# rapidsai/cugraph

Measured on NVIDIA B200. Metric: MTEPS (million traversed edges/sec) PageRank RMAT-24 ef-16, 100 iterations, higher is better.
Workload: dtype f32

## Files before the change

### cugraph_b200/csrc/pagerank.cu

```cuda
#include "sweep.cuh"

#include <algorithm>
#include <cmath>
#include <cstring>

namespace b200 {
namespace {

constexpr int kBlock = 256;
inline int grid_for(int64_t n) { return (int)std::min<int64_t>(std::max<int64_t>((n + kBlock - 1) / kBlock, 1), 1 << 22); }

template <typename T>
__global__ void k_fill(T* a, int32_t n, T v)
{
  int i = blockIdx.x * blockDim.x + threadIdx.x;
  if (i < n) a[i] = v;
}

__global__ void k_out_degree(int32_t const* __restrict__ indices, long long nnz, int32_t* __restrict__ deg)
{
  for (long long i = blockIdx.x * (long long)blockDim.x + threadIdx.x; i < nnz; i += (long long)gridDim.x * blockDim.x)
    atomicAdd(deg + indices[i], 1);
}

template <typename T>
__global__ void k_out_weight(int32_t const* __restrict__ indices, T const* __restrict__ w, long long nnz, double* __restrict__ sums)
{
  for (long long i = blockIdx.x * (long long)blockDim.x + threadIdx.x; i < nnz; i += (long long)gridDim.x * blockDim.x)
    atomicAdd(sums + indices[i], (double)w[i]);
}

template <typename S, typename T>
__global__ void k_cast(S const* in, int32_t n, T* out)
{
  int i = blockIdx.x * blockDim.x + threadIdx.x;
  if (i < n) out[i] = (T)in[i];
}

__device__ __forceinline__ double block_sum(double v, double* smem)
{
  v = warp_sum(v);
  if ((threadIdx.x & 31) == 0) smem[threadIdx.x >> 5] = v;
  __syncthreads();
  double t = 0.0;
  if (threadIdx.x < 32) {
    t = (threadIdx.x < (blockDim.x >> 5)) ? smem[threadIdx.x] : 0.0;
    t = warp_sum(t);
  }
  __syncthreads();
  return t;
}

template <typename T>
__global__ void __launch_bounds__(kBlock)
k_vertex_pass(T const* __restrict__ pr_new, T const* __restrict__ pr_old, T const* __restrict__ out_w,
              T* __restrict__ x, int32_t n, pr_state_t* __restrict__ st)
{
  if (st->done) return;
  __shared__ double smem[8];
  double diff = 0.0, dang = 0.0;
  for (int i = blockIdx.x * blockDim.x + threadIdx.x; i < n; i += gridDim.x * blockDim.x) {
    T nv = pr_new[i];
    T ow = out_w[i];
    if (pr_old) diff += fabs((double)nv - (double)pr_old[i]);
    if (ow == (T)0) dang += (double)nv;
    x[i] = (ow == (T)0) ? nv : nv / ow;
  }
  diff = block_sum(diff, smem);
  dang = block_sum(dang, smem);
  if (threadIdx.x == 0) {
    if (pr_old) atomicAdd(&st->diff, diff);
    atomicAdd(&st->dangling, dang);
  }
}

__global__ void k_finalize(pr_state_t* st, double alpha, double epsilon, int n_vertices, int personalized,
                           int count_iteration, int max_iterations)
{
  if (st->done) return;
  double base    = st->dangling * alpha + (1.0 - alpha);
  st->init       = personalized ? 0.0 : base / (double)n_vertices;
  st->pers_scale = base;
  if (count_iteration) {
    st->iter += 1;
    st->last_diff = st->diff;
    if (st->diff < epsilon || st->iter >= max_iterations) st->done = 1;
  }
  st->diff     = 0.0;
  st->dangling = 0.0;
}

template <typename T>
__global__ void k_personalize(int32_t const* __restrict__ pv, T const* __restrict__ pvals, int32_t n, double pers_sum,
                              T* __restrict__ y, pr_state_t const* __restrict__ st)
{
  if (st->done) return;
  int i = blockIdx.x * blockDim.x + threadIdx.x;
  if (i < n) y[pv[i]] = (T)((double)y[pv[i]] + st->pers_scale * ((double)pvals[i] / pers_sum));
}

template <typename T>
__global__ void k_sum(T const* a, int32_t n, double* out)
{
  __shared__ double smem[8];
  double s = 0.0;
  for (int i = blockIdx.x * blockDim.x + threadIdx.x; i < n; i += gridDim.x * blockDim.x) s += (double)a[i];
  s = block_sum(s, smem);
  if (threadIdx.x == 0) atomicAdd(out, s);
}

template <typename T>
__global__ void k_count_negative(T const* a, int64_t n, int* out)
{
  for (int64_t i = blockIdx.x * (int64_t)blockDim.x + threadIdx.x; i < n; i += (int64_t)gridDim.x * blockDim.x)
    if (a[i] < (T)0) atomicAdd(out, 1);
}

template <typename T>
__global__ void k_fill_pattern(T* x, int32_t n)
{
  int i = blockIdx.x * blockDim.x + threadIdx.x;
  if (i < n) x[i] = (T)(0.5 + (double)((unsigned)(i * 2654435761u) >> 16) / 65536.0);
}

template <typename O, typename T>
__global__ void k_compare_rows(O const* __restrict__ off, int32_t const* __restrict__ row_vertex, T const* __restrict__ a,
                               T const* __restrict__ b, int32_t n_rows, int32_t n_hi, double tol,
                               unsigned long long* __restrict__ worst , unsigned long long* __restrict__ n_bad )
{
  int r = blockIdx.x * blockDim.x + threadIdx.x;
  if (r >= n_rows) return;
  const int v        = row_vertex ? row_vertex[r] : r;
  const double va = (double)a[v], vb = (double)b[v];
  const double den   = fmax(fabs(va), 1e-300);
  const float rel    = (float)fmin(fabs(va - vb) / den, 1e30);
  const int cls      = r < n_hi ? 0 : 1;
  atomicMax(worst + cls, ((unsigned long long)__float_as_uint(rel) << 32) | (unsigned)r);
  if (rel > tol) atomicAdd(n_bad + cls, 1ull);
  (void)off;
}

struct pr_args {
  device_array_view_impl const* pre_v{nullptr};
  device_array_view_impl const* pre_w{nullptr};
  device_array_view_impl const* init_v{nullptr};
  device_array_view_impl const* init_val{nullptr};
  device_array_view_impl const* pers_v{nullptr};
  device_array_view_impl const* pers_val{nullptr};
  double alpha{0.85};
  double epsilon{1e-5};
  size_t max_iterations{100};
  bool expensive{false};
};

template <typename T>
void pagerank_typed(handle_impl const& h, graph_impl& g, pr_args const& a, centrality_result_impl& res)
{
  phase_trace tr(h);
  const int32_t nv = g.n_vertices;
  B200_EXPECTS(a.alpha >= 0.0 && a.alpha <= 1.0, CUGRAPH_UNKNOWN_ERROR, "Invalid input argument: alpha should be in [0.0, 1.0].");
  B200_EXPECTS(a.epsilon >= 0.0, CUGRAPH_UNKNOWN_ERROR, "Invalid input argument: epsilon should be non-negative.");
  if (nv == 0) {
    res.vertices   = new device_array_impl{dbuf(0, h.stream), 0, g.vertex_type};
    res.values     = new device_array_impl{dbuf(0, h.stream), 0, g.weight_type};
    res.iterations = 0;
    res.converged  = true;
    return;
  }
  csx_t const& c = pull_view(h, g);
  B200_EXPECTS(c.degree_sorted, CUGRAPH_UNKNOWN_ERROR, "internal: pull view is not binned");
  const bool weighted = g.weighted;

  dbuf out_w_user;
  T const* out_w = nullptr;
  if (a.pre_w) {
    out_w_user = collect_vertex_values<T>(h, g, a.pre_v, a.pre_w, (T)0);
    out_w      = out_w_user.as<T>();
  } else {
    if (c.out_w.data() == nullptr) {
      dbuf ow = make_dbuf<T>(nv, h.stream);
      if (weighted) {
        dbuf sums = make_dbuf<double>(nv, h.stream);
        CUDA_TRY(cudaMemsetAsync(sums.data(), 0, sizeof(double) * nv, h.stream));
        if (c.nnz > 0)
          B200_LAUNCH(h, (k_out_weight<T>), std::min(grid_for(c.nnz), 148 * 16), kBlock, 0, c.indices.as<int32_t>(),
                      c.weights.as<T>(), (long long)c.nnz, sums.as<double>());
        B200_LAUNCH(h, (k_cast<double, T>), grid_for(nv), kBlock, 0, sums.as<double>(), nv, ow.as<T>());
      } else {
        dbuf deg = make_dbuf<int32_t>(nv, h.stream);
        CUDA_TRY(cudaMemsetAsync(deg.data(), 0, sizeof(int32_t) * nv, h.stream));
        if (c.nnz > 0)
          B200_LAUNCH(h, k_out_degree, std::min(grid_for(c.nnz), 148 * 16), kBlock, 0, c.indices.as<int32_t>(),
                      (long long)c.nnz, deg.as<int32_t>());
        B200_LAUNCH(h, (k_cast<int32_t, T>), grid_for(nv), kBlock, 0, deg.as<int32_t>(), nv, ow.as<T>());
      }
      sync(h);
      c.out_w = std::move(ow);
    }
    out_w = c.out_w.as<T>();
  }
  tr.mark("pagerank: pull view + out-weights");
  if (a.expensive && weighted && c.nnz > 0) {
    dbuf neg = make_dbuf<int>(1, h.stream);
    CUDA_TRY(cudaMemsetAsync(neg.data(), 0, sizeof(int), h.stream));
    B200_LAUNCH(h, (k_count_negative<T>), std::min(grid_for(c.nnz), 148 * 16), kBlock, 0, c.weights.as<T>(), c.nnz, neg.as<int>());
    int hneg = 0;
    CUDA_TRY(cudaMemcpyAsync(&hneg, neg.data(), sizeof(int), cudaMemcpyDeviceToHost, h.stream));
    sync(h);
    B200_EXPECTS(hneg == 0, CUGRAPH_UNKNOWN_ERROR, "Invalid input argument: input edge weights should have non-negative values.");
  }

  dbuf pers_idx, pers_vals;
  int32_t n_pers  = 0;
  double pers_sum = 0.0;
  if (a.pers_v) {
    B200_EXPECTS(a.pers_val && a.pers_v->size == a.pers_val->size, CUGRAPH_UNKNOWN_ERROR,
                 "Invalid input argument: if personalization.has_value() is true, the size of vertices and values should match");
    B200_EXPECTS(a.pers_v->size > 0, CUGRAPH_UNKNOWN_ERROR,
                 "Invalid input argument: if personalizations.has_value() is true, the input personalization vector size should not be 0.");
    n_pers   = (int32_t)a.pers_v->size;
    pers_idx = make_dbuf<int32_t>(n_pers, h.stream);
    ext_to_int(h, g, a.pers_v->data, n_pers, pers_idx.as<int32_t>());
    dbuf bad = make_dbuf<int>(1, h.stream);
    CUDA_TRY(cudaMemsetAsync(bad.data(), 0, sizeof(int), h.stream));
    B200_LAUNCH(h, (k_count_negative<int32_t>), grid_for(n_pers), kBlock, 0, pers_idx.as<int32_t>(), (int64_t)n_pers, bad.as<int>());
    dbuf dsum = make_dbuf<double>(1, h.stream);
    CUDA_TRY(cudaMemsetAsync(dsum.data(), 0, sizeof(double), h.stream));
    B200_LAUNCH(h, (k_sum<T>), std::min(grid_for(n_pers), 1024), kBlock, 0, (T const*)a.pers_val->data, n_pers, dsum.as<double>());
    int hbad = 0;
    CUDA_TRY(cudaMemcpyAsync(&hbad, bad.data(), sizeof(int), cudaMemcpyDeviceToHost, h.stream));
    CUDA_TRY(cudaMemcpyAsync(&pers_sum, dsum.data(), sizeof(double), cudaMemcpyDeviceToHost, h.stream));
    sync(h);
    B200_EXPECTS(hbad == 0, CUGRAPH_INVALID_INPUT, "Invalid input argument: peresonalization vertices have invalid vertex IDs.");
    B200_EXPECTS(pers_sum > 0.0, CUGRAPH_UNKNOWN_ERROR, "Invalid input argument: sum of personalization valuese should be positive.");
  }

  dbuf pr_a = make_dbuf<T>(nv, h.stream), pr_b = make_dbuf<T>(nv, h.stream);
  dbuf x    = make_dbuf<T>(padded_x_elems(nv, sizeof(T)), h.stream);
  CUDA_TRY(cudaMemsetAsync(x.data(), 0, padded_x_elems(nv, sizeof(T)) * sizeof(T), h.stream));
  dbuf acc_hi = make_dbuf<double>(acc_rows(c), h.stream);
  CUDA_TRY(cudaMemsetAsync(acc_hi.data(), 0, sizeof(double) * acc_rows(c), h.stream));
  dbuf state = make_dbuf<pr_state_t>(1, h.stream);
  CUDA_TRY(cudaMemsetAsync(state.data(), 0, sizeof(pr_state_t), h.stream));
  pr_state_t* st = state.as<pr_state_t>();

  if (a.init_val) {
    dbuf guess = collect_vertex_values<T>(h, g, a.init_v, a.init_val, (T)0);
    CUDA_TRY(cudaMemcpyAsync(pr_a.data(), guess.data(), sizeof(T) * nv, cudaMemcpyDeviceToDevice, h.stream));
    sync(h);
  } else {
    B200_LAUNCH(h, (k_fill<T>), grid_for(nv), kBlock, 0, pr_a.as<T>(), nv, (T)((T)1 / (T)nv));
  }

  tr.mark("pagerank: state setup");
  const int vgrid = std::min(grid_for(nv), h.sm_count * 8);
  const int max_it = (int)std::min<size_t>(a.max_iterations, 0x7fffffff);
  B200_LAUNCH(h, (k_vertex_pass<T>), vgrid, kBlock, 0, pr_a.as<T>(), (T const*)nullptr, out_w, x.as<T>(), nv, st);
  B200_LAUNCH(h, k_finalize, 1, 1, 0, st, a.alpha, a.epsilon, nv, n_pers > 0 ? 1 : 0, 0, max_it);

  T* cur = pr_a.as<T>();
  T* nxt = pr_b.as<T>();
  pr_state_t* hst = reinterpret_cast<pr_state_t*>(h.pinned);
  int enqueued    = 0;
  int iters       = 0;
  const int batch = (a.epsilon > 0.0) ? 8 : 64;
  if (max_it == 0) {
  }
  while (true) {
    int todo = std::min(batch, std::max(max_it, 1) - enqueued);
    for (int k = 0; k < todo; ++k) {
      if (c.offs64) launch_pull_sweep<int64_t, T>(h, c, x.as<T>(), nxt, acc_hi.as<double>(), a.alpha, st);
      else launch_pull_sweep_auto<int32_t, T>(h, c, nv, x.as<T>(), nxt, acc_hi.as<double>(), a.alpha, st);
      if (n_pers > 0)
        B200_LAUNCH(h, (k_personalize<T>), grid_for(n_pers), kBlock, 0, pers_idx.as<int32_t>(), (T const*)a.pers_val->data,
                    n_pers, pers_sum, nxt, st);
      B200_LAUNCH(h, (k_vertex_pass<T>), vgrid, kBlock, 0, nxt, cur, out_w, x.as<T>(), nv, st);
      B200_LAUNCH(h, k_finalize, 1, 1, 0, st, a.alpha, a.epsilon, nv, n_pers > 0 ? 1 : 0, 1, max_it);
      std::swap(cur, nxt);
      ++enqueued;
    }
    check_last("pagerank iteration");
    CUDA_TRY(cudaMemcpyAsync(hst, st, sizeof(pr_state_t), cudaMemcpyDeviceToHost, h.stream));
    sync(h);
    iters = hst->iter;
    if (hst->done || enqueued >= std::max(max_it, 1)) break;
  }
  tr.mark("pagerank: iterations (+ layout staging on the first call)");
  T* final_pr = (iters % 2 == 0) ? pr_a.as<T>() : pr_b.as<T>();

  res.vertices   = new device_array_impl{reported_vertices(h, g), (size_t)nv, g.vertex_type};
  res.values     = new device_array_impl{to_reported_order(h, g, final_pr, sizeof(T)), (size_t)nv, g.weight_type};
  res.iterations = (size_t)iters;
  res.converged  = (size_t)iters < a.max_iterations;
  sync(h);
  tr.mark("pagerank: result gather");
}

cugraph_error_code_t pagerank_entry(const cugraph_resource_handle_t* handle, cugraph_graph_t* graph, pr_args a,
                                    bool require_convergence, cugraph_centrality_result_t** result,
                                    cugraph_error_t** error)
{
  return guarded(error, [&] {
    auto const& h = H(handle);
    auto* g       = G(graph);
    B200_EXPECTS(result != nullptr, CUGRAPH_INVALID_INPUT, "result out-pointer is NULL");
    *result = nullptr;
    if (a.pre_v) {
      B200_EXPECTS(a.pre_v->type == g->vertex_type, CUGRAPH_INVALID_INPUT,
                   "vertex type of graph and precomputed_vertex_out_weight_vertices must match");
      B200_EXPECTS(a.pre_w && a.pre_w->type == g->weight_type, CUGRAPH_INVALID_INPUT,
                   "vertex type of graph and precomputed_vertex_out_weight_sums must match");
    }
    if (a.init_v) {
      B200_EXPECTS(a.init_v->type == g->vertex_type, CUGRAPH_INVALID_INPUT,
                   "vertex type of graph and initial_guess_vertices must match");
      B200_EXPECTS(a.init_val && a.init_val->type == g->weight_type, CUGRAPH_INVALID_INPUT,
                   "vertex type of graph and initial_guess_values must match");
    }
    if (a.pers_v) {
      B200_EXPECTS(a.pers_v->type == g->vertex_type, CUGRAPH_INVALID_INPUT,
                   "vertex type of graph and personalization_vector must match");
      B200_EXPECTS(a.pers_val && a.pers_val->type == g->weight_type, CUGRAPH_INVALID_INPUT,
                   "vertex type of graph and personalization_vector must match");
    }
    if (!a.pre_w) a.pre_v = nullptr;
    if (!a.init_val) a.init_v = nullptr;
    auto res = std::make_unique<centrality_result_impl>();
    if (g->mg) {
      mg_pagerank(h, *g, mg_pr_args{a.alpha, a.epsilon, a.max_iterations}, *res);
    } else if (g->weight_type == FLOAT32) {
      pagerank_typed<float>(h, *g, a, *res);
    } else {
      pagerank_typed<double>(h, *g, a, *res);
    }
    bool converged = res->converged;
    *result        = reinterpret_cast<cugraph_centrality_result_t*>(res.release());
    B200_EXPECTS(!require_convergence || converged, CUGRAPH_UNKNOWN_ERROR, "PageRank failed to converge.");
  });
}

}

}

using namespace b200;

extern "C" {

cugraph_type_erased_device_array_view_t* cugraph_centrality_result_get_vertices(cugraph_centrality_result_t* result)
{
  auto* r = reinterpret_cast<centrality_result_impl*>(result);
  return reinterpret_cast<cugraph_type_erased_device_array_view_t*>(r->vertices->new_view());
}

cugraph_type_erased_device_array_view_t* cugraph_centrality_result_get_values(cugraph_centrality_result_t* result)
{
  auto* r = reinterpret_cast<centrality_result_impl*>(result);
  return reinterpret_cast<cugraph_type_erased_device_array_view_t*>(r->values->new_view());
}

size_t cugraph_centrality_result_get_num_iterations(cugraph_centrality_result_t* result)
{
  return reinterpret_cast<centrality_result_impl*>(result)->iterations;
}

bool_t cugraph_centrality_result_converged(cugraph_centrality_result_t* result)
{
  return reinterpret_cast<centrality_result_impl*>(result)->converged ? TRUE : FALSE;
}

void cugraph_centrality_result_free(cugraph_centrality_result_t* result)
{
  if (!result) return;
  auto* r = reinterpret_cast<centrality_result_impl*>(result);
  delete r->vertices;
  delete r->values;
  delete r;
}

#define PR_ARGS_COMMON                                                                          \
  pr_args a;                                                                                    \
  a.pre_v          = V(precomputed_vertex_out_weight_vertices);                                 \
  a.pre_w          = V(precomputed_vertex_out_weight_sums);                                     \
  a.init_v         = V(initial_guess_vertices);                                                 \
  a.init_val       = V(initial_guess_values);                                                   \
  a.alpha          = alpha;                                                                     \
  a.epsilon        = epsilon;                                                                   \
  a.max_iterations = max_iterations;                                                            \
  a.expensive      = do_expensive_check == TRUE;

cugraph_error_code_t cugraph_pagerank(const cugraph_resource_handle_t* handle, cugraph_graph_t* graph,
                                      const cugraph_type_erased_device_array_view_t* precomputed_vertex_out_weight_vertices,
                                      const cugraph_type_erased_device_array_view_t* precomputed_vertex_out_weight_sums,
                                      const cugraph_type_erased_device_array_view_t* initial_guess_vertices,
                                      const cugraph_type_erased_device_array_view_t* initial_guess_values, double alpha,
                                      double epsilon, size_t max_iterations, bool_t do_expensive_check,
                                      cugraph_centrality_result_t** result, cugraph_error_t** error)
{
  PR_ARGS_COMMON
  return pagerank_entry(handle, graph, a, true, result, error);
}

cugraph_error_code_t cugraph_pagerank_allow_nonconvergence(
  const cugraph_resource_handle_t* handle, cugraph_graph_t* graph,
  const cugraph_type_erased_device_array_view_t* precomputed_vertex_out_weight_vertices,
  const cugraph_type_erased_device_array_view_t* precomputed_vertex_out_weight_sums,
  const cugraph_type_erased_device_array_view_t* initial_guess_vertices,
  const cugraph_type_erased_device_array_view_t* initial_guess_values, double alpha, double epsilon,
  size_t max_iterations, bool_t do_expensive_check, cugraph_centrality_result_t** result, cugraph_error_t** error)
{
  PR_ARGS_COMMON
  return pagerank_entry(handle, graph, a, false, result, error);
}

cugraph_error_code_t cugraph_personalized_pagerank(
  const cugraph_resource_handle_t* handle, cugraph_graph_t* graph,
  const cugraph_type_erased_device_array_view_t* precomputed_vertex_out_weight_vertices,
  const cugraph_type_erased_device_array_view_t* precomputed_vertex_out_weight_sums,
  const cugraph_type_erased_device_array_view_t* initial_guess_vertices,
  const cugraph_type_erased_device_array_view_t* initial_guess_values,
  const cugraph_type_erased_device_array_view_t* personalization_vertices,
  const cugraph_type_erased_device_array_view_t* personalization_values, double alpha, double epsilon,
  size_t max_iterations, bool_t do_expensive_check, cugraph_centrality_result_t** result, cugraph_error_t** error)
{
  PR_ARGS_COMMON
  a.pers_v   = V(personalization_vertices);
  a.pers_val = V(personalization_values);
  return pagerank_entry(handle, graph, a, true, result, error);
}

// ... 106 lines not shown
```

### cugraph_b200/csrc/spmv.cuh

```cuda
#pragma once
#include "graph.cuh"

#include <cstdlib>

namespace b200 {

struct pr_state_t {
  double diff;
  double dangling;
  double init;
  double pers_scale;
  double last_diff;
  int iter;
  int done;
};

#ifndef B200_HOST_EMU
__device__ __forceinline__ int ld_stream(const int* p)
{
  int v;
  asm volatile("ld.global.nc.L1::no_allocate.s32 %0, [%1];" : "=r"(v) : "l"(p));
  return v;
}
__device__ __forceinline__ float ld_stream(const float* p)
{
  float v;
  asm volatile("ld.global.nc.L1::no_allocate.f32 %0, [%1];" : "=f"(v) : "l"(p));
  return v;
}
__device__ __forceinline__ double ld_stream(const double* p)
{
  double v;
  asm volatile("ld.global.nc.L1::no_allocate.f64 %0, [%1];" : "=d"(v) : "l"(p));
  return v;
}
#else
inline int ld_stream(const int* p) { return *p; }
inline float ld_stream(const float* p) { return *p; }
inline double ld_stream(const double* p) { return *p; }
#endif

__device__ __forceinline__ double warp_sum(double v)
{
#pragma unroll
  for (int o = 16; o > 0; o >>= 1) v += __shfl_xor_sync(0xffffffffu, v, o);
  return v;
}

template <typename O, typename T, bool WEIGHTED>
__global__ void __launch_bounds__(256)
k_spmv_hi(O const* __restrict__ offsets, int32_t const* __restrict__ indices, T const* __restrict__ weights,
          T const* __restrict__ x, T* __restrict__ y, int32_t const* __restrict__ row_vertex,
          int32_t const* __restrict__ chunk_first_row, int32_t n_chunks, long long nnz_hi,
          double* __restrict__ acc_hi, double alpha, pr_state_t const* __restrict__ st)
{
  if (st->done) return;
  const int lane = threadIdx.x & 31;
  const int c    = (int)((blockIdx.x * (long long)blockDim.x + threadIdx.x) >> 5);
  if (c >= n_chunks) return;
  const double init  = st->init;
  const long long e0 = (long long)c * kWarpChunk;
  const long long e1 = (e0 + kWarpChunk < nnz_hi) ? e0 + kWarpChunk : nnz_hi;
  int r              = chunk_first_row[c];
  long long row_beg  = (long long)offsets[r];
  long long row_end  = (long long)offsets[r + 1];
  long long e        = e0;
  while (e < e1) {
    const long long seg_end = row_end < e1 ? row_end : e1;
    double acc              = 0.0;
    long long i             = e + lane;
    for (; i + 96 < seg_end; i += 128) {
      int s0 = ld_stream(indices + i), s1 = ld_stream(indices + i + 32);
      int s2 = ld_stream(indices + i + 64), s3 = ld_stream(indices + i + 96);
      T x0 = x[s0], x1 = x[s1], x2 = x[s2], x3 = x[s3];
      if (WEIGHTED) {
        x0 *= ld_stream(weights + i);
        x1 *= ld_stream(weights + i + 32);
        x2 *= ld_stream(weights + i + 64);
        x3 *= ld_stream(weights + i + 96);
      }
      acc += ((double)x0 + (double)x1) + ((double)x2 + (double)x3);
    }
    for (; i < seg_end; i += 32) {
      T xv = x[ld_stream(indices + i)];
      if (WEIGHTED) xv *= ld_stream(weights + i);
      acc += (double)xv;
    }
    acc = warp_sum(acc);
    if (lane == 0) {
      const bool whole = (row_beg >= e0) && (row_end <= e1);
      if (whole) {
        const int v = row_vertex ? row_vertex[r] : r;
        y[v]        = (T)(acc * alpha + init);
      } else {
        atomicAdd(acc_hi + r, acc);
      }
    }
    e = seg_end;
    if (e == row_end && e < e1) {
      ++r;
      row_beg = row_end;
      row_end = (long long)offsets[r + 1];
    }
  }
}

template <typename T>
__global__ void k_spmv_hi_finish(int32_t const* __restrict__ split_rows, int32_t n_split, double* __restrict__ acc_hi,
                                 T* __restrict__ y, int32_t const* __restrict__ row_vertex, double alpha,
                                 pr_state_t const* __restrict__ st)
{
  if (st->done) return;
  int k = blockIdx.x * blockDim.x + threadIdx.x;
  if (k >= n_split) return;
  int r     = split_rows[k];
  int v     = row_vertex ? row_vertex[r] : r;
  y[v]      = (T)(acc_hi[r] * alpha + st->init);
  acc_hi[r] = 0.0;
}

struct low_bins_t {
  int32_t row_begin[kNumSeg];
  int32_t block_begin[kNumSeg];
};

__host__ __device__ __forceinline__ int low_bin_lanes(int b) { return b == 0 ? 4 : (b == 1 ? 2 : 1); }

template <typename O, typename T, bool WEIGHTED>
__global__ void __launch_bounds__(256)
k_spmv_low(O const* __restrict__ offsets, int32_t const* __restrict__ indices, T const* __restrict__ weights,
           T const* __restrict__ x, T* __restrict__ y, int32_t const* __restrict__ row_vertex, low_bins_t bins,
           double alpha, pr_state_t const* __restrict__ st)
{
  if (st->done) return;
  int b = 0;
#pragma unroll
  for (int k = 1; k < kNumSeg - 1; ++k)
    if ((int)blockIdx.x >= bins.block_begin[k]) b = k;
  const double init = st->init;
  const int blk     = blockIdx.x - bins.block_begin[b];
  if (b == kNumSeg - 2) {
    int r = bins.row_begin[b] + blk * 256 + threadIdx.x;
    if (r < bins.row_begin[b + 1]) y[row_vertex ? row_vertex[r] : r] = (T)init;
    return;
  }
  const int g   = low_bin_lanes(b);
  const int sub = threadIdx.x & (g - 1);
  const int r   = bins.row_begin[b] + blk * (256 / g) + (threadIdx.x / g);
  double acc    = 0.0;
  const bool in = r < bins.row_begin[b + 1];
  if (in) {
    const long long lo = (long long)offsets[r], hi = (long long)offsets[r + 1];
    constexpr int kR = 8;
    int c[kR];
    T wv[kR];
#pragma unroll
    for (int k = 0; k < kR; ++k) {
      const long long e = lo + sub + (long long)k * g;
      c[k]              = 0;
      wv[k]             = (T)0;
      if (e < hi) {
        c[k]  = __ldg(indices + e);
        wv[k] = WEIGHTED ? __ldg(weights + e) : (T)1;
      }
    }
    T v[kR];
#pragma unroll
// ... 57 lines not shown
```

### cugraph_b200/csrc/sweep.cuh

```cuda
#pragma once
#include "spmv.cuh"

namespace b200 {



constexpr int kSweepThreads = 512;
constexpr int kSweepWarps   = kSweepThreads / 32;
constexpr int kSweepDynSmem = kHotSliceBytes;
constexpr int kTmaPiece     = 16 * 1024;
constexpr int kStealMin     = 12;

#ifndef B200_HOST_EMU
__device__ __forceinline__ uint32_t smem_u32(const void* p) { return (uint32_t)__cvta_generic_to_shared(p); }

__device__ __forceinline__ void mbar_init(uint64_t* bar, unsigned count)
{
  asm volatile("mbarrier.init.shared::cta.b64 [%0], %1;" ::"r"(smem_u32(bar)), "r"(count));
  asm volatile("fence.mbarrier_init.release.cluster;" ::: "memory");
}
__device__ __forceinline__ void mbar_expect_tx(uint64_t* bar, unsigned bytes)
{
  asm volatile("mbarrier.arrive.expect_tx.shared::cta.b64 _, [%0], %1;" ::"r"(smem_u32(bar)), "r"(bytes) : "memory");
}
// ... 390 lines not shown
    if (j == cnt_cur && cnt_cur > 0) {
      slot ^= 1;
      if (lane < kDrawMax) ring[slot * kDrawMax + lane] = pend;
      __syncwarp();
      cnt_cur = cnt_nxt;
      j       = 0;
      const int b2 = draw_get(raw_nn);
      cnt_nxt      = b2 < n ? (n - b2 < want_nn ? n - b2 : want_nn) : 0;
      pend         = batch_headers(chunks, b2, cnt_nxt, lane);
      const int w3 = draw_want(n, b2 < n ? b2 + want_nn : n);
      raw_nn       = draw_issue(cursor, w3, lane, b2 + want_nn < n);
      want_nn      = w3;
    }
    sweep_chunk_t ch;
    ch.kind = -1;
    ch.n_groups = ch.sr_begin = ch.row_begin = 0;
    if (cnt_cur > 0) {
      const uint4 h = ring[slot * kDrawMax + j];
      ++j;
      ch.sr_begin  = (int)h.x;
      ch.row_begin = (int)h.y;
      ch.n_groups  = (int)h.z;
      ch.kind      = (int)h.w;
    }
    return ch;
  }
};

template <typename T, bool WEIGHTED>
__global__ void __launch_bounds__(kSweepThreads, 1) k_sweep(sweep_args_t<T> a)
{
  B200_DYN_SMEM(smem_raw);
  T* sx = reinterpret_cast<T*>(smem_raw);
  __shared__ uint64_t bar;
  __shared__ int s_best;
  __shared__ uint4 s_ring[kSweepWarps][2 * kDrawMax];
  if (a.st->done) return;
  a.p.pol        = make_l2_policy_evict_first();
  a.p.acc_pol    = make_l2_policy_evict_last();
  const int lane = threadIdx.x & 31;
  const int me   = (int)blockIdx.x;
  if (threadIdx.x == 0) mbar_init(&bar, 1);
  if (threadIdx.x < kHotZeroPad) sx[a.W + threadIdx.x] = (T)0;
  const int own_lo = a.cta_phase[me], own_hi = a.cta_phase[me + 1];
  int next_own    = own_lo;
  unsigned parity = 0;
  int cur_block   = -1;
  while (true) {
    int p = -1;
    if (next_own < own_hi) {
      p = next_own++;
    } else {
      if (threadIdx.x == 0) s_best = 0;
      __syncthreads();
      int best = 0;
      for (int q = (int)threadIdx.x; q < a.n_phases; q += kSweepThreads) {
        if (q >= own_lo && q < own_hi) continue;
        const sweep_phase_t ph = a.phases[q];
        const int left         = (ph.chunk_end - ph.chunk_begin) - ld_volatile(a.cursor + q);
        if (left >= kStealMin && left > best) best = left;
      }
      if (best > 0) atomicMax(&s_best, best);
      __syncthreads();
      const int win = s_best;
      __syncthreads();
      if (win > 0) {
        if (threadIdx.x == 0) s_best = a.n_phases;
        __syncthreads();
        for (int q = (int)threadIdx.x; q < a.n_phases; q += kSweepThreads) {
          if (q >= own_lo && q < own_hi) continue;
          const sweep_phase_t ph = a.phases[q];
          const int left         = (ph.chunk_end - ph.chunk_begin) - ld_volatile(a.cursor + q);
          if (left >= kStealMin && left * 2 >= win) atomicMin(&s_best, q);
        }
        __syncthreads();
        p = s_best < a.n_phases ? s_best : -1;
      }
    }
    __syncthreads();
    if (p < 0) break;
    const sweep_phase_t ph = a.phases[p];
    const int n            = ph.chunk_end - ph.chunk_begin;
    const bool fresh       = ph.block != cur_block;
    if (fresh) {
      if (threadIdx.x == 0) {
        const unsigned bytes = (unsigned)(a.W * sizeof(T));
        mbar_expect_tx(&bar, bytes);
        const unsigned char* src = reinterpret_cast<const unsigned char*>(a.x + (size_t)ph.block * a.W);
        for (unsigned o = 0; o < bytes; o += kTmaPiece)
          tma_bulk_g2s(smem_raw + o, src + o, (bytes - o) < (unsigned)kTmaPiece ? (bytes - o) : (unsigned)kTmaPiece, &bar);
      }
      cur_block = ph.block;
    }
    chunk_supply_t sup;
    sup.start(a.chunks + ph.chunk_begin, a.cursor + p, s_ring[threadIdx.x >> 5], n, lane);
    sweep_chunk_t hA = sup.next(lane);
    sweep_chunk_t hB = sup.next(lane);
    chunk_regs_t A, B;
    chunk_load(A, hA, a.p, lane);
    if (fresh) {
      mbar_wait(&bar, parity);
      parity ^= 1;
    }
    while (hA.kind >= 0) {
      chunk_load(B, hB, a.p, lane);
      const sweep_chunk_t hC = sup.next(lane);
      chunk_process<T, WEIGHTED>(A, hA, a.p, sx, lane);
      if (hB.kind < 0) break;
      chunk_load(A, hC, a.p, lane);
      const sweep_chunk_t hD = sup.next(lane);
      chunk_process<T, WEIGHTED>(B, hB, a.p, sx, lane);
      hA = hC;
      hB = hD;
    }
  }
}

template <typename T, int kFinishSteps>
__global__ void __launch_bounds__(256)
k_sweep_finish(double* __restrict__ acc, int n_cov, int n_rows, T* __restrict__ y, int32_t const* __restrict__ row_vertex,
               double alpha, int* __restrict__ cursor, int n_phases, pr_state_t const* __restrict__ st)
{
  if (st->done) return;
  const int t = blockIdx.x * blockDim.x + threadIdx.x;
  if (t < n_phases) cursor[t] = 0;
  const int lane = threadIdx.x & 31;
  const int base = (t >> 5) * (64 * kFinishSteps) + 2 * lane;
  if (base - 2 * lane >= n_rows) return;
  const double init = st->init;
  double2 q[kFinishSteps];
#pragma unroll
  for (int k = 0; k < kFinishSteps; ++k) {
    const int r = base + 64 * k;
    q[k]        = make_double2(0.0, 0.0);
    if (r + 1 < n_cov) q[k] = *reinterpret_cast<double2*>(acc + r);
    else if (r < n_cov) q[k].x = acc[r];
  }
#pragma unroll
  for (int k = 0; k < kFinishSteps; ++k) {
    const int r = base + 64 * k;
    if (r + 1 < n_cov) *reinterpret_cast<double2*>(acc + r) = make_double2(0.0, 0.0);
    else if (r < n_cov) acc[r] = 0.0;
    const T v0 = (T)(q[k].x * alpha + init), v1 = (T)(q[k].y * alpha + init);
    if (!row_vertex && r + 1 < n_rows && sizeof(T) == 4) {
      *reinterpret_cast<float2*>(y + r) = make_float2((float)v0, (float)v1);
    } else {
      if (r < n_rows) y[row_vertex ? row_vertex[r] : r] = v0;
      if (r + 1 < n_rows) y[row_vertex ? row_vertex[r + 1] : r + 1] = v1;
    }
  }
}

template <typename T>
void launch_sweep(handle_impl const& h, csx_t const& c, sweep_layout_t const& L, T const* x, T* y, double* acc, double alpha,
                  pr_state_t const* st, bool use_weights = true, bool covered_rows_only = false)
{
  const bool weighted = use_weights && L.w.data() != nullptr;
  if (weighted) CUDA_TRY(cudaFuncSetAttribute(k_sweep<T, true>, cudaFuncAttributeMaxDynamicSharedMemorySize, kSweepDynSmem));
  else CUDA_TRY(cudaFuncSetAttribute(k_sweep<T, false>, cudaFuncAttributeMaxDynamicSharedMemorySize, kSweepDynSmem));
  sweep_args_t<T> a;
  a.p.ids     = L.ids.as<uint4>();
  a.p.rows    = L.rows.as<int32_t>();
  a.p.w       = L.w.data();
  a.p.acc     = acc;
  a.chunks    = L.chunks.as<sweep_chunk_t>();
  a.phases    = L.phases.as<sweep_phase_t>();
  a.cta_phase = L.cta_phase.as<int32_t>();
  a.cursor    = L.cursor.as<int>();
  a.x         = x;
  a.st        = st;
  a.n_phases  = L.n_phases;
  a.W         = L.W;
  a.p.pol     = 0;
  a.p.acc_pol = 0;
  if (weighted) B200_LAUNCH(h, (k_sweep<T, true>), L.n_cta, kSweepThreads, kSweepDynSmem, a);
  else B200_LAUNCH(h, (k_sweep<T, false>), L.n_cta, kSweepThreads, kSweepDynSmem, a);
  constexpr int kFinishSteps = 8;
  const int32_t finish_rows = covered_rows_only ? L.n_cov : c.n_rows;
  const int n = std::max((finish_rows + 2 * kFinishSteps - 1) / (2 * kFinishSteps), L.n_phases);
  B200_LAUNCH(h, (k_sweep_finish<T, kFinishSteps>), (n + 255) / 256, 256, 0, acc, L.n_cov, finish_rows, y, c.row_vertex.as<int32_t>(), alpha,
              L.cursor.as<int>(), L.n_phases, st);
}

template <typename O, typename T>
void launch_pull_sweep_auto(handle_impl const& h, csx_t const& c, int32_t n_vertices, T const* x, T* y, double* acc,
                            double alpha, pr_state_t const* st, bool use_weights = true, bool covered_rows_only = false)
{
  sweep_layout_t const* L = sweep_layout(h, c, n_vertices, sizeof(T));
  if (!L) launch_pull_sweep<O, T>(h, c, x, y, acc, alpha, st, use_weights);
  else launch_sweep<T>(h, c, *L, x, y, acc, alpha, st, use_weights, covered_rows_only);
}

inline size_t padded_x_elems(int32_t n_vertices, size_t elem_size)
{
  const size_t slice = kHotSliceBytes / elem_size;
  const size_t W     = slice - kHotZeroPad;
  return ((size_t)n_vertices / W + 2) * slice;
}

}
```

### emu/cuda_runtime.h

```cpp
#pragma once
#ifndef B200_HOST_EMU
#error "emu/cuda_runtime.h is only for -DB200_HOST_EMU builds"
#endif
#include <algorithm>
#include <chrono>
#include <climits>
#include <cmath>
#include <cstdint>
#include <cstdio>
#include <cstdlib>
#include <cstring>

#define __global__
#define __device__
#define __host__
#define __forceinline__ inline
#define __launch_bounds__(...)
#define __shared__ static

struct uint3 { unsigned x{0}, y{0}, z{0}; };
struct dim3 {
  unsigned x{1}, y{1}, z{1};
  dim3(unsigned a = 1, unsigned b = 1, unsigned c = 1) : x(a), y(b), z(c) {}
};
// ... 146 lines not shown
  yield_to_scheduler();
  for (int i = 0; i < 32; ++i) out[i] = W.out[i];
  return W.out_mask;
}

}

template <typename F>
inline void emu_launch(long long grid, long long block, F&& body)
{
  if (block > emu::kMaxThreads) { std::fprintf(stderr, "emu: block of %lld threads\n", block); std::abort(); }
  gridDim        = dim3((unsigned)grid);
  blockDim       = dim3((unsigned)block);
  emu::cta().body = [&] { body(); };
  for (long long b = 0; b < grid; ++b) {
    blockIdx.x = (unsigned)b;
    emu::run_cta((int)block);
  }
}

typedef int cudaError_t;
enum { cudaSuccess = 0, cudaErrorMemoryAllocation = 2 };
typedef struct emu_stream_t* cudaStream_t;
typedef struct emu_event_t* cudaEvent_t;
typedef void* cudaMemPool_t;
enum cudaMemcpyKind { cudaMemcpyHostToHost, cudaMemcpyHostToDevice, cudaMemcpyDeviceToHost, cudaMemcpyDeviceToDevice, cudaMemcpyDefault };
enum { cudaStreamNonBlocking = 1, cudaEventDisableTiming = 2 };
enum cudaMemPoolAttr { cudaMemPoolAttrReleaseThreshold = 4 };
enum cudaFuncAttribute { cudaFuncAttributeMaxDynamicSharedMemorySize = 8 };
struct cudaDeviceProp {
  int multiProcessorCount{4};
  int l2CacheSize{1 << 20};
};

inline const char* cudaGetErrorString(cudaError_t) { return "emulated CUDA error"; }
inline const char* cudaGetErrorName(cudaError_t) { return "cudaErrorEmu"; }
inline cudaError_t cudaGetLastError() { return cudaSuccess; }
inline cudaError_t cudaGetDevice(int* d) { *d = 0; return cudaSuccess; }
inline cudaError_t cudaGetDeviceProperties(cudaDeviceProp* p, int) { *p = cudaDeviceProp{}; return cudaSuccess; }
inline cudaError_t cudaDeviceGetDefaultMemPool(cudaMemPool_t* p, int) { *p = nullptr; return cudaSuccess; }
inline cudaError_t cudaMemPoolSetAttribute(cudaMemPool_t, cudaMemPoolAttr, void*) { return cudaSuccess; }
inline cudaError_t cudaMalloc(void** p, size_t n) { *p = std::malloc(n ? n : 1); return *p ? cudaSuccess : cudaErrorMemoryAllocation; }
template <typename T> inline cudaError_t cudaMalloc(T** p, size_t n) { return cudaMalloc((void**)p, n); }
inline cudaError_t cudaMallocAsync(void** p, size_t n, cudaStream_t) { return cudaMalloc(p, n); }
template <typename T> inline cudaError_t cudaMallocAsync(T** p, size_t n, cudaStream_t s) { return cudaMallocAsync((void**)p, n, s); }
inline cudaError_t cudaMallocHost(void** p, size_t n) { return cudaMalloc(p, n); }
template <typename T> inline cudaError_t cudaMallocHost(T** p, size_t n) { return cudaMalloc((void**)p, n); }
inline cudaError_t cudaFree(void* p) { std::free(p); return cudaSuccess; }
inline cudaError_t cudaFreeAsync(void* p, cudaStream_t) { std::free(p); return cudaSuccess; }
inline cudaError_t cudaFreeHost(void* p) { std::free(p); return cudaSuccess; }
inline cudaError_t cudaMemcpy(void* d, const void* s, size_t n, cudaMemcpyKind) { if (n) std::memmove(d, s, n); return cudaSuccess; }
inline cudaError_t cudaMemcpyAsync(void* d, const void* s, size_t n, cudaMemcpyKind k, cudaStream_t = nullptr) { return cudaMemcpy(d, s, n, k); }
inline cudaError_t cudaMemset(void* d, int v, size_t n) { if (n) std::memset(d, v, n); return cudaSuccess; }
inline cudaError_t cudaMemsetAsync(void* d, int v, size_t n, cudaStream_t = nullptr) { return cudaMemset(d, v, n); }
inline cudaError_t cudaStreamCreateWithFlags(cudaStream_t* s, unsigned) { *s = (cudaStream_t)std::malloc(8); return cudaSuccess; }
inline cudaError_t cudaStreamCreate(cudaStream_t* s) { return cudaStreamCreateWithFlags(s, 0); }
inline cudaError_t cudaStreamDestroy(cudaStream_t s) { std::free(s); return cudaSuccess; }
inline cudaError_t cudaStreamSynchronize(cudaStream_t) { return cudaSuccess; }
inline cudaError_t cudaStreamWaitEvent(cudaStream_t, cudaEvent_t, unsigned = 0) { return cudaSuccess; }
inline cudaError_t cudaEventCreateWithFlags(cudaEvent_t* e, unsigned) { *e = (cudaEvent_t)std::malloc(8); return cudaSuccess; }
inline cudaError_t cudaEventCreate(cudaEvent_t* e) { return cudaEventCreateWithFlags(e, 0); }
inline cudaError_t cudaEventDestroy(cudaEvent_t e) { std::free(e); return cudaSuccess; }
inline cudaError_t cudaEventRecord(cudaEvent_t e, cudaStream_t = nullptr)
{
  const double t = std::chrono::duration<double, std::milli>(std::chrono::steady_clock::now().time_since_epoch()).count();
  std::memcpy(e, &t, sizeof(t));
  return cudaSuccess;
}
inline cudaError_t cudaEventSynchronize(cudaEvent_t) { return cudaSuccess; }
inline cudaError_t cudaDeviceSynchronize() { return cudaSuccess; }
inline cudaError_t cudaEventElapsedTime(float* ms, cudaEvent_t a, cudaEvent_t b)
{
  double ta, tb;
  std::memcpy(&ta, a, sizeof(ta));
  std::memcpy(&tb, b, sizeof(tb));
  *ms = (float)(tb - ta);
  return cudaSuccess;
}
template <typename F> inline cudaError_t cudaFuncSetAttribute(F, cudaFuncAttribute, int) { return cudaSuccess; }

template <typename T> inline T atomicAdd(T* p, T v) { T o = *p; *p = o + v; return o; }
template <typename T> inline T atomicMin(T* p, T v) { T o = *p; if (v < o) *p = v; return o; }
template <typename T> inline T atomicMax(T* p, T v) { T o = *p; if (v > o) *p = v; return o; }
template <typename T> inline T atomicOr(T* p, T v) { T o = *p; *p = o | v; return o; }
inline unsigned __float_as_uint(float f) { unsigned u; std::memcpy(&u, &f, 4); return u; }
inline float __uint_as_float(unsigned u) { float f; std::memcpy(&f, &u, 4); return f; }
inline long long __double_as_longlong(double d) { long long u; std::memcpy(&u, &d, 8); return u; }
template <typename T> inline T __ldg(const T* p) { return *p; }
template <typename T> inline unsigned long long emu_bits(T v) { unsigned long long b = 0; static_assert(sizeof(T) <= 8, "shuffle width"); std::memcpy(&b, &v, sizeof(T)); return b; }
template <typename T> inline T emu_from_bits(unsigned long long b) { T v; std::memcpy(&v, &b, sizeof(T)); return v; }
inline int emu_lane() { return (int)(threadIdx.x & 31); }
template <typename T> inline T emu_shfl_from(unsigned mask, T v, int src)
{
  unsigned long long out[32];
  const unsigned pm = emu::warp_collect(mask, emu_bits(v), out);
  if (src < 0 || src > 31 || !((pm >> src) & 1u)) src = emu_lane();
  return emu_from_bits<T>(out[src]);
}
template <typename T> inline T __shfl_sync(unsigned m, T v, int src, int width = 32)
{
  return emu_shfl_from(m, v, (src & (width - 1)) + (emu_lane() & ~(width - 1)));
}
template <typename T> inline T __shfl_xor_sync(unsigned m, T v, int o, int = 32) { return emu_shfl_from(m, v, emu_lane() ^ o); }
template <typename T> inline T __shfl_down_sync(unsigned m, T v, int o, int = 32) { return emu_shfl_from(m, v, emu_lane() + o); }
template <typename T> inline T __shfl_up_sync(unsigned m, T v, int o, int = 32) { return emu_shfl_from(m, v, emu_lane() - o); }
inline unsigned __ballot_sync(unsigned m, int p)
{
  unsigned long long out[32];
  const unsigned pm = emu::warp_collect(m, p ? 1ull : 0ull, out);
  unsigned r = 0;
  for (int i = 0; i < 32; ++i)
    if (((pm >> i) & 1u) && out[i]) r |= 1u << i;
  return r;
}
inline int __all_sync(unsigned m, int p)
{
  unsigned long long out[32];
  const unsigned pm = emu::warp_collect(m, p ? 1ull : 0ull, out);
  for (int i = 0; i < 32; ++i)
    if (((pm >> i) & 1u) && !out[i]) return 0;
  return 1;
}
inline int __any_sync(unsigned m, int p) { return __ballot_sync(m, p) != 0; }
template <typename T> inline unsigned __match_any_sync(unsigned m, T v)
{
  unsigned long long out[32];
  const unsigned pm = emu::warp_collect(m, emu_bits(v), out);
  const unsigned long long mine = emu_bits(v);
  unsigned r = 0;
  for (int i = 0; i < 32; ++i)
    if (((pm >> i) & 1u) && out[i] == mine) r |= 1u << i;
  return r;
}
inline unsigned __reduce_or_sync(unsigned m, unsigned v)
{
  unsigned long long out[32];
  const unsigned pm = emu::warp_collect(m, (unsigned long long)v, out);
  unsigned r = 0;
  for (int i = 0; i < 32; ++i)
    if ((pm >> i) & 1u) r |= (unsigned)out[i];
  return r;
}
template <typename T> inline T __reduce_add_sync(unsigned m, T v)
{
  unsigned long long out[32];
  const unsigned pm = emu::warp_collect(m, emu_bits(v), out);
  T r = 0;
  for (int i = 0; i < 32; ++i)
    if ((pm >> i) & 1u) r += emu_from_bits<T>(out[i]);
  return r;
}
inline unsigned __activemask() { return 1u << emu_lane(); }
inline void __syncwarp(unsigned m = 0xffffffffu) { unsigned long long out[32]; emu::warp_collect(m, 0ull, out); }
inline void __syncthreads()
{
  emu::cta_state_t& C = emu::cta();
  if (!C.in_fiber) return;
  C.state[C.cur] = emu::WAIT_CTA;
  ++C.cta_arrived;
  emu::yield_to_scheduler();
}
inline int __popc(unsigned v) { return __builtin_popcount(v); }
inline int __popcll(unsigned long long v) { return __builtin_popcountll(v); }
inline int __ffsll(long long v) { return __builtin_ffsll(v); }
inline int __ffs(int v) { return __builtin_ffs(v); }
inline int __clz(int v) { return v ? __builtin_clz((unsigned)v) : 32; }
inline float __int_as_float(int i) { float f; std::memcpy(&f, &i, 4); return f; }
inline int __float_as_int(float f) { int i; std::memcpy(&i, &f, 4); return i; }
inline double __longlong_as_double(long long i) { double f; std::memcpy(&f, &i, 8); return f; }
template <typename T> inline T atomicExch(T* p, T v) { T o = *p; *p = v; return o; }
template <typename T> inline T atomicCAS(T* p, T c, T v) { T o = *p; if (o == c) *p = v; return o; }
```

Measured before the change: 738,200.

## Fuse sweep finish, vertex pass and state finalize into one PageRank kernel

For the common non-personalized, 32-bit-offset, full-row layout path, the per-iteration sweep finish kernel, the vertex pass and the single-thread finalize kernel are replaced by one fused kernel. That kernel turns the double accumulator into the new ranks, clears the accumulator, computes x and the diff/dangling sums with vectorized loads, and resets the phase cursors. The last block to finish, found through an atomic ticket, advances the convergence state. This removes two kernel launches and one full pass over the vertex arrays per iteration. In exchange it relies on correct fencing in the last-block pattern and adds a new ticket field to the state struct.

```diff
diff --git a/cugraph_b200/csrc/pagerank.cu b/cugraph_b200/csrc/pagerank.cu
--- a/cugraph_b200/csrc/pagerank.cu
+++ b/cugraph_b200/csrc/pagerank.cu
@@ -74,20 +74,117 @@
   }
 }
 
-__global__ void k_finalize(pr_state_t* st, double alpha, double epsilon, int n_vertices, int personalized,
-                           int count_iteration, int max_iterations)
-{
-  if (st->done) return;
-  double base    = st->dangling * alpha + (1.0 - alpha);
+__device__ __forceinline__ void advance_state(pr_state_t* st, double diff, double dangling, double alpha, double epsilon,
+                                              int n_vertices, int personalized, int count_iteration, int max_iterations)
+{
+  double base    = dangling * alpha + (1.0 - alpha);
   st->init       = personalized ? 0.0 : base / (double)n_vertices;
   st->pers_scale = base;
   if (count_iteration) {
     st->iter += 1;
-    st->last_diff = st->diff;
-    if (st->diff < epsilon || st->iter >= max_iterations) st->done = 1;
+    st->last_diff = diff;
+    if (diff < epsilon || st->iter >= max_iterations) st->done = 1;
   }
   st->diff     = 0.0;
   st->dangling = 0.0;
+}
+
+__global__ void k_finalize(pr_state_t* st, double alpha, double epsilon, int n_vertices, int personalized,
+                           int count_iteration, int max_iterations)
+{
+  if (st->done) return;
+  advance_state(st, st->diff, st->dangling, alpha, epsilon, n_vertices, personalized, count_iteration, max_iterations);
+}
+
+template <typename T> struct vec2_of;
+template <> struct vec2_of<float> { using type = float2; };
+template <> struct vec2_of<double> { using type = double2; };
+
+template <typename T>
+constexpr int pr_steps() { return 16 / (int)sizeof(T); }
+constexpr int kPrCtasPerSm = 3;
+
+template <typename T>
+__global__ void __launch_bounds__(256, kPrCtasPerSm)
+k_pagerank_finish(double* __restrict__ acc, int n_cov, int n_rows, T* __restrict__ pr_new, T const* __restrict__ pr_old,
+                  T const* __restrict__ out_w, T* __restrict__ x, int* __restrict__ cursor, int n_phases, double alpha,
+                  double epsilon, int max_iterations, pr_state_t* __restrict__ st)
+{
+  using T2 = typename vec2_of<T>::type;
+  constexpr int kPrSteps = pr_steps<T>();
+  __shared__ double s_red[2][8];
+  if (st->done) return;
+  for (int i = blockIdx.x * blockDim.x + threadIdx.x; i < n_phases; i += gridDim.x * blockDim.x) cursor[i] = 0;
+  const int lane    = threadIdx.x & 31;
+  const int n_warps = gridDim.x * (blockDim.x >> 5);
+  const int n_tiles = (n_rows + 64 * kPrSteps - 1) / (64 * kPrSteps);
+  const double init = st->init;
+  double diff = 0.0, dang = 0.0;
+  for (int tile = blockIdx.x * (blockDim.x >> 5) + (threadIdx.x >> 5); tile < n_tiles; tile += n_warps) {
+    const int base = tile * (64 * kPrSteps) + 2 * lane;
+    double2 q[kPrSteps];
+    T2 old[kPrSteps], ow[kPrSteps];
+#pragma unroll
+    for (int k = 0; k < kPrSteps; ++k) {
+      const int r = base + 64 * k;
+      q[k]        = make_double2(0.0, 0.0);
+      if (r + 1 < n_cov) q[k] = *reinterpret_cast<double2 const*>(acc + r);
+      else if (r < n_cov) q[k].x = acc[r];
+      old[k] = T2{(T)0, (T)0};
+      ow[k]  = T2{(T)0, (T)0};
+      if (r + 1 < n_rows) {
+        old[k] = *reinterpret_cast<T2 const*>(pr_old + r);
+        ow[k]  = *reinterpret_cast<T2 const*>(out_w + r);
+      } else if (r < n_rows) {
+        old[k].x = pr_old[r];
+        ow[k].x  = out_w[r];
+      }
+    }
+#pragma unroll
+    for (int k = 0; k < kPrSteps; ++k) {
+      const int r = base + 64 * k;
+      if (r + 1 < n_cov) *reinterpret_cast<double2*>(acc + r) = make_double2(0.0, 0.0);
+      else if (r < n_cov) acc[r] = 0.0;
+      if (r >= n_rows) continue;
+      const T v0 = (T)(q[k].x * alpha + init), v1 = (T)(q[k].y * alpha + init);
+      const T x0 = (ow[k].x == (T)0) ? v0 : v0 / ow[k].x, x1 = (ow[k].y == (T)0) ? v1 : v1 / ow[k].y;
+      diff += fabs((double)v0 - (double)old[k].x);
+      if (ow[k].x == (T)0) dang += (double)v0;
+      if (r + 1 < n_rows) {
+        diff += fabs((double)v1 - (double)old[k].y);
+        if (ow[k].y == (T)0) dang += (double)v1;
+        *reinterpret_cast<T2*>(pr_new + r) = T2{v0, v1};
+        *reinterpret_cast<T2*>(x + r)      = T2{x0, x1};
+      } else {
+        pr_new[r] = v0;
+        x[r]      = x0;
+      }
+    }
+  }
+  diff = warp_sum(diff);
+  dang = warp_sum(dang);
+  if (lane == 0) {
+    s_red[0][threadIdx.x >> 5] = diff;
+    s_red[1][threadIdx.x >> 5] = dang;
+  }
+  __syncthreads();
+  if (threadIdx.x == 0) {
+    double d = 0.0, g = 0.0;
+    for (int w = 0; w < (int)(blockDim.x >> 5); ++w) {
+      d += s_red[0][w];
+      g += s_red[1][w];
+    }
+    atomicAdd(&st->diff, d);
+    atomicAdd(&st->dangling, g);
+    __threadfence();
+    if (atomicAdd(&st->ticket, 1u) == gridDim.x - 1) {
+      __threadfence();
+      volatile pr_state_t const* vs = st;
+      const double sum_diff = vs->diff, sum_dang = vs->dangling;
+      advance_state(st, sum_diff, sum_dang, alpha, epsilon, n_rows, 0, 1, max_iterations);
+      st->ticket = 0;
+    }
+  }
 }
 
 template <typename T>
@@ -266,16 +363,25 @@
   const int batch = (a.epsilon > 0.0) ? 8 : 64;
   if (max_it == 0) {
   }
+  sweep_layout_t const* L = (!c.offs64 && n_pers == 0 && c.row_vertex.data() == nullptr && c.n_rows == nv)
+                              ? sweep_layout(h, c, nv, sizeof(T)) : nullptr;
+  const int fin_grid = std::max(std::min(ceil_div(nv, 64 * pr_steps<T>() * 8), h.sm_count * kPrCtasPerSm), 1);
   while (true) {
     int todo = std::min(batch, std::max(max_it, 1) - enqueued);
     for (int k = 0; k < todo; ++k) {
-      if (c.offs64) launch_pull_sweep<int64_t, T>(h, c, x.as<T>(), nxt, acc_hi.as<double>(), a.alpha, st);
-      else launch_pull_sweep_auto<int32_t, T>(h, c, nv, x.as<T>(), nxt, acc_hi.as<double>(), a.alpha, st);
-      if (n_pers > 0)
-        B200_LAUNCH(h, (k_personalize<T>), grid_for(n_pers), kBlock, 0, pers_idx.as<int32_t>(), (T const*)a.pers_val->data,
-                    n_pers, pers_sum, nxt, st);
-      B200_LAUNCH(h, (k_vertex_pass<T>), vgrid, kBlock, 0, nxt, cur, out_w, x.as<T>(), nv, st);
-      B200_LAUNCH(h, k_finalize, 1, 1, 0, st, a.alpha, a.epsilon, nv, n_pers > 0 ? 1 : 0, 1, max_it);
+      if (L) {
+        launch_sweep_pieces<T>(h, *L, x.as<T>(), acc_hi.as<double>(), st);
+        B200_LAUNCH(h, (k_pagerank_finish<T>), fin_grid, 256, 0, acc_hi.as<double>(), L->n_cov, nv, nxt,
+                    (T const*)cur, out_w, x.as<T>(), L->cursor.as<int>(), L->n_phases, a.alpha, a.epsilon, max_it, st);
+      } else {
+        if (c.offs64) launch_pull_sweep<int64_t, T>(h, c, x.as<T>(), nxt, acc_hi.as<double>(), a.alpha, st);
+        else launch_pull_sweep_auto<int32_t, T>(h, c, nv, x.as<T>(), nxt, acc_hi.as<double>(), a.alpha, st);
+        if (n_pers > 0)
+          B200_LAUNCH(h, (k_personalize<T>), grid_for(n_pers), kBlock, 0, pers_idx.as<int32_t>(), (T const*)a.pers_val->data,
+                      n_pers, pers_sum, nxt, st);
+        B200_LAUNCH(h, (k_vertex_pass<T>), vgrid, kBlock, 0, nxt, cur, out_w, x.as<T>(), nv, st);
+        B200_LAUNCH(h, k_finalize, 1, 1, 0, st, a.alpha, a.epsilon, nv, n_pers > 0 ? 1 : 0, 1, max_it);
+      }
       std::swap(cur, nxt);
       ++enqueued;
     }
diff --git a/cugraph_b200/csrc/spmv.cuh b/cugraph_b200/csrc/spmv.cuh
--- a/cugraph_b200/csrc/spmv.cuh
+++ b/cugraph_b200/csrc/spmv.cuh
@@ -13,6 +13,7 @@
   double last_diff;
   int iter;
   int done;
+  unsigned ticket;
 };
 
 #ifndef B200_HOST_EMU
diff --git a/cugraph_b200/csrc/sweep.cuh b/cugraph_b200/csrc/sweep.cuh
--- a/cugraph_b200/csrc/sweep.cuh
+++ b/cugraph_b200/csrc/sweep.cuh
@@ -566,8 +566,8 @@
 }
 
 template <typename T>
-void launch_sweep(handle_impl const& h, csx_t const& c, sweep_layout_t const& L, T const* x, T* y, double* acc, double alpha,
-                  pr_state_t const* st, bool use_weights = true, bool covered_rows_only = false)
+void launch_sweep_pieces(handle_impl const& h, sweep_layout_t const& L, T const* x, double* acc, pr_state_t const* st,
+                         bool use_weights = true)
 {
   const bool weighted = use_weights && L.w.data() != nullptr;
   if (weighted) CUDA_TRY(cudaFuncSetAttribute(k_sweep<T, true>, cudaFuncAttributeMaxDynamicSharedMemorySize, kSweepDynSmem));
@@ -589,6 +589,13 @@
   a.p.acc_pol = 0;
   if (weighted) B200_LAUNCH(h, (k_sweep<T, true>), L.n_cta, kSweepThreads, kSweepDynSmem, a);
   else B200_LAUNCH(h, (k_sweep<T, false>), L.n_cta, kSweepThreads, kSweepDynSmem, a);
+}
+
+template <typename T>
+void launch_sweep(handle_impl const& h, csx_t const& c, sweep_layout_t const& L, T const* x, T* y, double* acc, double alpha,
+                  pr_state_t const* st, bool use_weights = true, bool covered_rows_only = false)
+{
+  launch_sweep_pieces<T>(h, L, x, acc, st, use_weights);
   constexpr int kFinishSteps = 8;
   const int32_t finish_rows = covered_rows_only ? L.n_cov : c.n_rows;
   const int n = std::max((finish_rows + 2 * kFinishSteps - 1) / (2 * kFinishSteps), L.n_phases);
diff --git a/emu/cuda_runtime.h b/emu/cuda_runtime.h
--- a/emu/cuda_runtime.h
+++ b/emu/cuda_runtime.h
@@ -322,6 +322,7 @@
 }
 inline unsigned __activemask() { return 1u << emu_lane(); }
 inline void __syncwarp(unsigned m = 0xffffffffu) { unsigned long long out[32]; emu::warp_collect(m, 0ull, out); }
+inline void __threadfence() {}
 inline void __syncthreads()
 {
   emu::cta_state_t& C = emu::cta();
```

After: 769,900 (median of 6 runs). 4.3% higher.
